# LuoweiZhou/VLP

Measured on NVIDIA H100. Metric: image_text_samples_per_sec, higher is better.
Workload: dtype bf16

## Files before the change

include/vlpk.h:

```cpp
#ifndef VLPK_H_
#define VLPK_H_

#include <stddef.h>
#include <stdint.h>

#ifdef __cplusplus
extern "C" {
#endif

#define VLPK_VERSION 102

#define VLPK_BF16 0
#define VLPK_F32 1
#define VLPK_I64 2
#define VLPK_MASK_ADDITIVE 0
#define VLPK_MASK_ZERO_ONE 1
#define VLPK_ACT_NONE 0
#define VLPK_ACT_RELU 1

typedef struct VlpkDropout {
  float p;
  uint64_t seed;
  const uint64_t* seed_dev;
} VlpkDropout;
// ... 27 lines not shown
typedef struct VlpkLayerActs {
  void* qkv;
  void* ctx;
  void* t1;
  void* y1;
  void* u;
  void* hmid;
  void* t2;
  void* y;
  float* lse;
  float* stats1;
  float* stats2;
  void* kv;
  unsigned char* drop_attn;
} VlpkLayerActs;

typedef struct VlpkBwdScratch {
  void* dz2;
  void* dt2;
  void* du;
  void* dy1;
  void* dz1;
  void* dt1;
  void* dctx;
  void* dqkv;
  void* dx;
} VlpkBwdScratch;

int vlpk_version(void);
const char* vlpk_last_error(void);
void vlpk_set_reserved_sms(int n);
void vlpk_set_deterministic(int on);
int vlpk_debug_plan_gemm(int M, int N, int K, int a_mn, int b_mn, int nseg, int seg_rows, int epi, int bn, int splits, int* out2);
int vlpk_debug_set_option(const char* name, int value);

int vlpk_mask_pack(const void* mask, int dtype, int mode, int B, int rows, int kv, int64_t stride_b, int64_t stride_r,
                   uint32_t* out, void* stream);

int vlpk_mask_synth(const int32_t* len_b, const int32_t* mode, int len_a, int B, int L, uint32_t* out, void* stream);

int vlpk_linear_fwd(int M, int N, int K, const void* x, int64_t ldx, const void* w, int64_t ldw, const void* bias, void* y,
                    int64_t ldy, int act, const VlpkDropout* drop, uint64_t site, void* stream);
int vlpk_linear_bwd(int M, int N, int K, const void* x, int64_t ldx, const void* w, int64_t ldw, const void* y, int64_t ldy,
                    const void* dy, int64_t lddy, void* dpre, void* dx, int64_t lddx, float* dw, int64_t lddw, float* db,
                    int act, float p_drop, void* stream);

int vlpk_embed_fwd(int B, int L, int H, int R, int vis_input, const int64_t* ids, const int64_t* token_type, const int64_t* pos,
                   const void* word_w, const void* pos_w, const void* type_w, const void* vis, const void* vis_pe,
                   const void* ln_g, const void* ln_b, void* y, float* stats, const VlpkDropout* drop, uint64_t site, void* stream);
int vlpk_embed_bwd(int B, int L, int H, int R, int vis_input, const int64_t* ids, const int64_t* token_type, const int64_t* pos,
                   const void* word_w, const void* pos_w, const void* type_w, const void* vis, const void* vis_pe,
                   const void* ln_g, const float* stats, const void* dy, void* dz, float* d_ln_g, float* d_ln_b,
                   const VlpkDropout* drop, uint64_t site, void* stream);

int vlpk_embed_tables_bwd(int B, int L, int H, int R, int vis_input, const int64_t* ids, const int64_t* token_type, const int64_t* pos,
                          const void* dz, int V, int P, int T, void* d_word, float* word_scratch, float* d_pos, float* d_type,
                          void* stream);

int vlpk_ln_res_drop_fwd(int64_t M, int H, const void* t, const void* res, const void* gamma, const void* beta, void* y,
                         float* stats, const VlpkDropout* drop, uint64_t site, void* stream);
int vlpk_ln_res_drop_bwd(int64_t M, int H, const void* t, const void* res, const void* gamma, const float* stats, const void* dy,
                         void* dz, void* dt, float* dgamma, float* dbeta, float* dbias, const VlpkDropout* drop, uint64_t site,
                         void* stream);

int vlpk_attn_core_fwd(int B, int heads, int Lq, int Lkv, const void* q, int64_t ld_q, const void* k, const void* v, int64_t ld_kv,
                       const uint32_t* mask_bits, int mask_rows, void* ctx, int64_t ld_ctx, float* lse, const VlpkDropout* drop,
// ... 116 lines not shown
```

vlp_b200/_lib.py:

```python
import ctypes as C
import os

import torch

_HERE = os.path.dirname(os.path.abspath(__file__))
LIB_PATH = os.path.join(_HERE, "libvlpk.so")

c_void_p, c_int, c_i64, c_u64, c_float = C.c_void_p, C.c_int, C.c_int64, C.c_uint64, C.c_float


class VlpkDropout(C.Structure):
    _fields_ = [("p", c_float), ("seed", c_u64), ("seed_dev", c_void_p)]


class VlpkShape(C.Structure):
    _fields_ = [("B", C.c_int32), ("Lq", C.c_int32), ("Lkv", C.c_int32), ("H", C.c_int32), ("heads", C.c_int32),
                ("I", C.c_int32), ("kv_slots", C.c_int32)]


WEIGHT_FIELDS = ["wq", "wk", "wv", "bq", "bk", "bv", "wo", "bo", "ln1_g", "ln1_b", "w1", "b1", "w2", "b2", "ln2_g", "ln2_b"]
GRAD_FIELDS = ["wqkv", "bqkv", "wo", "bo", "ln1_g", "ln1_b", "w1", "b1", "w2", "b2", "ln2_g", "ln2_b"]
ACT_FIELDS = ["qkv", "ctx", "t1", "y1", "u", "hmid", "t2", "y", "lse", "stats1", "stats2", "kv", "drop_attn"]
SCRATCH_FIELDS = ["dz2", "dt2", "du", "dy1", "dz1", "dt1", "dctx", "dqkv", "dx"]


class VlpkLayerWeights(C.Structure):
    _fields_ = [(n, c_void_p) for n in WEIGHT_FIELDS]


class VlpkLayerGrads(C.Structure):
    _fields_ = [(n, c_void_p) for n in GRAD_FIELDS]


class VlpkLayerActs(C.Structure):
    _fields_ = [(n, c_void_p) for n in ACT_FIELDS]


class VlpkBwdScratch(C.Structure):
    _fields_ = [(n, c_void_p) for n in SCRATCH_FIELDS]


class VlpkAdamTensor(C.Structure):
    _fields_ = [("param", c_void_p), ("grad", c_void_p), ("master", c_void_p), ("m", c_void_p), ("v", c_void_p), ("n", c_i64),
                ("weight_decay", c_float), ("param_dtype", C.c_int32), ("grad_dtype", C.c_int32), ("reserved", C.c_int32)]


_P = c_void_p
_SIGS = {
    "vlpk_version": (c_int, []),
    "vlpk_last_error": (C.c_char_p, []),
    "vlpk_debug_set_option": (c_int, [C.c_char_p, c_int]),
    "vlpk_set_reserved_sms": (None, [c_int]),
    "vlpk_set_deterministic": (None, [c_int]),
    "vlpk_debug_plan_gemm": (c_int, [c_int] * 10 + [C.POINTER(c_int)]),
    "vlpk_mask_pack": (c_int, [_P, c_int, c_int, c_int, c_int, c_int, c_i64, c_i64, _P, _P]),
    "vlpk_mask_synth": (c_int, [_P, _P, c_int, c_int, c_int, _P, _P]),
    "vlpk_linear_fwd": (c_int, [c_int, c_int, c_int, _P, c_i64, _P, c_i64, _P, _P, c_i64, c_int, C.POINTER(VlpkDropout), c_u64, _P]),
    "vlpk_linear_bwd": (c_int, [c_int, c_int, c_int, _P, c_i64, _P, c_i64, _P, c_i64, _P, c_i64, _P, _P, c_i64, _P, c_i64, _P,
                                c_int, c_float, _P]),
    "vlpk_embed_fwd": (c_int, [c_int, c_int, c_int, c_int, c_int, _P, _P, _P, _P, _P, _P, _P, _P, _P, _P, _P, _P,
                               C.POINTER(VlpkDropout), c_u64, _P]),
    "vlpk_embed_bwd": (c_int, [c_int, c_int, c_int, c_int, c_int, _P, _P, _P, _P, _P, _P, _P, _P, _P, _P, _P, _P, _P, _P,
                               C.POINTER(VlpkDropout), c_u64, _P]),
    "vlpk_embed_tables_bwd": (c_int, [c_int, c_int, c_int, c_int, c_int, _P, _P, _P, _P, c_int, c_int, c_int, _P, _P, _P, _P, _P]),
    "vlpk_ln_res_drop_fwd": (c_int, [c_i64, c_int, _P, _P, _P, _P, _P, _P, C.POINTER(VlpkDropout), c_u64, _P]),
    "vlpk_ln_res_drop_bwd": (c_int, [c_i64, c_int, _P, _P, _P, _P, _P, _P, _P, _P, _P, _P, C.POINTER(VlpkDropout), c_u64, _P]),
    "vlpk_attn_core_fwd": (c_int, [c_int, c_int, c_int, c_int, _P, c_i64, _P, _P, c_i64, _P, c_int, _P, c_i64, _P,
                                   C.POINTER(VlpkDropout), c_u64, _P]),
    "vlpk_attn_core_bwd": (c_int, [c_int, c_int, c_int, _P, _P, _P, c_i64, _P, c_int, _P, _P, c_i64, _P, _P, _P, _P, c_i64,
                                   C.POINTER(VlpkDropout), c_u64, _P]),
    "vlpk_attn_core_fwd_wide": (c_int, [c_int, c_int, c_int, c_int, _P, c_i64, _P, _P, c_i64, _P, c_int, _P, c_i64, _P,
                                        C.POINTER(VlpkDropout), c_u64, c_int, _P]),
    "vlpk_attn_core_bwd_wide": (c_int, [c_int, c_int, c_int, _P, _P, _P, c_i64, _P, c_int, _P, _P, c_i64, _P, _P, _P, _P, c_i64,
                                        C.POINTER(VlpkDropout), c_u64, c_int, _P]),
    "vlpk_attn_core_self_fwd": (c_int, [c_int, c_int, c_int, c_int, _P, c_i64, c_i64, _P, _P, c_i64, c_i64, _P, _P, _P, c_int, _P, c_i64,
                                        c_i64, _P, _P]),
    "vlpk_attn_core_group_self_fwd": (c_int, [c_int, c_int, c_int, c_int, c_int, c_int, _P, c_i64, c_i64, _P, c_int, c_i64, _P, c_int,
                                              c_i64, _P, _P, _P, c_int, _P, c_i64, c_i64, _P, _P]),
    "vlpk_attn_probs": (c_int, [c_int, c_int, c_int, c_int, c_int, _P, c_i64, c_i64, _P, c_i64, c_i64, _P, c_int, c_int, _P, _P, c_i64,
                                c_i64, _P]),
    "vlpk_mha_fwd": (c_int, [C.POINTER(VlpkShape), C.POINTER(VlpkLayerWeights), _P, _P, _P, c_int, C.POINTER(VlpkLayerActs),
                             c_float, c_float, C.POINTER(VlpkDropout), c_u64, _P]),
    "vlpk_ffn_fwd": (c_int, [C.POINTER(VlpkShape), C.POINTER(VlpkLayerWeights), C.POINTER(VlpkLayerActs), c_float,
                             C.POINTER(VlpkDropout), c_u64, _P]),
    "vlpk_layer_fwd": (c_int, [C.POINTER(VlpkShape), C.POINTER(VlpkLayerWeights), _P, _P, _P, c_int, C.POINTER(VlpkLayerActs),
                               c_float, c_float, C.POINTER(VlpkDropout), c_u64, _P]),
    "vlpk_layer_bwd": (c_int, [C.POINTER(VlpkShape), C.POINTER(VlpkLayerWeights), _P, _P, c_int, C.POINTER(VlpkLayerActs), _P, _P,
# ... 97 lines not shown
```

vlp_b200/csrc/api.cu:

```cuda
#include "../../include/vlpk.h"

#include <cstdlib>
#include <cstring>

#include "attn.cuh"
#include "decode.cuh"
#include "gemm.cuh"
#include "head.cuh"
#include "host.cuh"
#include "optim.cuh"
#include "rowops.cuh"
#include "tables.cuh"

using namespace vlpk;
typedef __nv_bfloat16 bf16;

namespace {

inline cudaStream_t S(void* s) { return reinterpret_cast<cudaStream_t>(s); }

enum { SITE_ATTN = 0, SITE_HID1 = 1, SITE_HID2 = 2 };
inline uint64_t site_of(uint64_t layer_id, int site) { return layer_id * 8 + site; }

inline DropoutCfg mk_drop(const VlpkDropout* d, float p, uint64_t site) {
// ... 372 lines not shown
  VlpkShape rows = *s;
  rows.Lq = rows.Lkv = R;
  VLPK_TRY(attn_out_ln(&rows, w, x, a, 0.f, nullptr, layer_id, st));
  return ffn_fwd_impl(&rows, w, a, 0.f, nullptr, layer_id, st);
}

int score_stack_fwd(const VlpkShape* s, int T, int n_layers, const VlpkLayerWeights* w, const void* x, AttnGroupKv* group,
                    const void* const* prefix, const uint32_t* key_bits, const uint32_t* query_bits, VlpkLayerActs* acts, cudaStream_t st) {
  const void* cur = x;
  for (int i = 0; i < n_layers; ++i) {
    if (group != nullptr) group->prefix = prefix[i];
    VLPK_TRY(score_layer_fwd(s, T, group, &w[i], cur, key_bits, query_bits, &acts[i], i, st));
    cur = acts[i].y;
  }
  return 0;
}

size_t act_bytes(const VlpkShape* s, size_t rows, size_t kv_elems) {
  const size_t H = s->H, I = s->I, M = static_cast<size_t>(s->B) * rows;
  const size_t lse = (static_cast<size_t>(s->B) * s->heads * rows + 3) / 4 * 4;
  return 2 * (M * (3 * H + 5 * H + 2 * I) + kv_elems) + 4 * (lse + 4 * M);
}

}

#pragma GCC visibility push(default)
extern "C" {

int vlpk_version(void) { return VLPK_VERSION; }
int vlpk_debug_set_option(const char* name, int value) {
  VLPK_CHECK_ARG(name != nullptr, "set_option: null name");
  if (strcmp(name, "wgrad_stream") == 0) { g_wgrad_stream = value ? 1 : 0; return 0; }
  if (strcmp(name, "attn_tiled") == 0) { set_attn_tiled(value != 0); return 0; }
  set_error("set_option: unknown option '%s'", name);
  return -1;
}
int vlpk_debug_plan_gemm(int M, int N, int K, int a_mn, int b_mn, int nseg, int seg_rows, int epi, int bn, int splits, int* out2) {
  GemmDesc g;
  g.M = M; g.N = N; g.K = K;
  g.a_mn = a_mn != 0; g.b_mn = b_mn != 0;
  g.nseg = nseg; g.b_seg_rows = seg_rows;
  g.epi = epi; g.bn = bn; g.splits = splits;
  return plan_gemm(g, &out2[0], &out2[1]);
}
void vlpk_set_reserved_sms(int n) { set_reserved_sms(n); }
void vlpk_set_deterministic(int on) { set_deterministic(on != 0); }
const char* vlpk_last_error(void) { return get_error(); }

int vlpk_mask_pack(const void* mask, int dtype, int mode, int B, int rows, int kv, int64_t stride_b, int64_t stride_r, uint32_t* out,
                   void* stream) {
  VLPK_CHECK_ARG(mask != nullptr && out != nullptr, "mask_pack: null pointer");
  return launch_mask_pack(mask, dtype, mode, B, rows, kv, stride_b, stride_r, out, S(stream));
}

int vlpk_mask_synth(const int32_t* len_b, const int32_t* mode, int len_a, int B, int L, uint32_t* out, void* stream) {
  return launch_mask_synth(len_b, mode, len_a, B, L, out, S(stream));
}

int vlpk_linear_fwd(int M, int N, int K, const void* x, int64_t ldx, const void* w, int64_t ldw, const void* bias, void* y, int64_t ldy,
                    int act, const VlpkDropout* drop, uint64_t site, void* stream) {
  VLPK_CHECK_ARG(x && w && y, "linear_fwd: null pointer");
  VLPK_CHECK_ARG(act == VLPK_ACT_NONE || act == VLPK_ACT_RELU, "linear_fwd: act %d unsupported", act);
  const DropoutCfg dc = (act == VLPK_ACT_RELU && drop != nullptr) ? mk_drop(drop, drop->p, site) : make_dropout(0.f, 0, site);
  return fwd_linear(M, N, K, x, ldx, w, ldw, bias, y, ldy, act == VLPK_ACT_RELU ? EPI_RELU : EPI_STORE, nullptr, 0, dc, S(stream));
}

int vlpk_linear_bwd(int M, int N, int K, const void* x, int64_t ldx, const void* w, int64_t ldw, const void* y, int64_t ldy,
                    const void* dy, int64_t lddy, void* dpre, void* dx, int64_t lddx, float* dw, int64_t lddw, float* db, int act,
                    float p_drop, void* stream) {
  VLPK_CHECK_ARG(x && w && dy && dw, "linear_bwd: null pointer");
  cudaStream_t st = S(stream);
  const void* g = dy;
  int64_t ldg = lddy;
  if (act == VLPK_ACT_RELU) {
    VLPK_CHECK_ARG(y != nullptr && dpre != nullptr && N % 8 == 0, "linear_bwd: relu needs y, dpre and N %% 8 == 0");
    const long long n = static_cast<long long>(M) * N;
// ... 516 lines not shown
```

vlp_b200/csrc/gemm.cu:

```cuda
#include "gemm.cuh"

#include <cstdlib>

#include "host.cuh"
#include "rowops.cuh"

namespace vlpk {

static constexpr int BM = 128;
static constexpr int BK = 64;
static constexpr int NUM_THREADS = 384;
static constexpr int PRODUCER_REGS = 24;
static constexpr int CONSUMER_REGS = 240;
static constexpr int STG_BYTES = 64 * 128;
static constexpr int STG_PER_CONSUMER = 4;
static constexpr int SMEM_MAX = 232448;
static constexpr int BN = 128;

struct GemmTmaps {
  CUtensorMap a;
  CUtensorMap b[3];
  CUtensorMap d0;
  CUtensorMap d1;
  CUtensorMap aux;
};

struct GemmArgs {
  int M, N, K;
  int b_seg_rows;
  int splits;
  int split_slices;
  const __nv_bfloat16* bias[3];
  float relu_scale;
  DropoutCfg drop;
  float* colsum;
};

template <int STAGES>
struct SmemLayout {
  static constexpr int A_BYTES = BM * BK * 2;
  static constexpr int B_BYTES = BN * BK * 2;
  static constexpr int STAGE_BYTES = A_BYTES + B_BYTES;
  static constexpr int OFF_STG = STAGES * STAGE_BYTES;
  static constexpr int OFF_BAR = OFF_STG + 2 * STG_PER_CONSUMER * STG_BYTES;
  static constexpr int NUM_BARS = 3 * STAGES + 2;
  static constexpr int TOTAL = OFF_BAR + NUM_BARS * 8;
  static constexpr int DYN_BYTES = TOTAL + 1024;
  static_assert(DYN_BYTES <= SMEM_MAX, "shared memory budget exceeded");
};

struct StageCount {
  static constexpr int value = (SMEM_MAX - 1024 - 2 * STG_PER_CONSUMER * STG_BYTES - 256) / (BM * BK * 2 + BN * BK * 2);
};

__device__ __forceinline__ void wg_bar_sync(int cw) {
  asm volatile("bar.sync %0, 128;" ::"r"(cw + 1) : "memory");
}

template <bool A_MN, bool B_MN, int EPI>
__global__ void __launch_bounds__(NUM_THREADS, 1)
gemm_kernel(const __grid_constant__ GemmTmaps tm, const GemmArgs args) {
  constexpr int STAGES = StageCount::value;
  using L = SmemLayout<STAGES>;
  extern __shared__ uint8_t smem_raw[];
  uint8_t* smem = reinterpret_cast<uint8_t*>((reinterpret_cast<uintptr_t>(smem_raw) + 1023) & ~uintptr_t(1023));

  uint64_t* bars = reinterpret_cast<uint64_t*>(smem + L::OFF_BAR);
  uint64_t* full_bar = bars;
  uint64_t* empty_bar = bars + 2 * STAGES;
  uint64_t* aux_bar = bars + 3 * STAGES;
  constexpr bool HAS_AUX = (EPI == EPI_ADD || EPI == EPI_MUL || EPI == EPI_DRELU);

  pdl_launch_dependents();
  const int wg = __shfl_sync(0xffffffffu, threadIdx.x >> 7, 0);
  const int lane = threadIdx.x & 31;

  const int num_m = (args.M + BM - 1) / BM;
  const int num_n = (args.N + BN - 1) / BN;
  const int total_kb = (args.K + BK - 1) / BK;
  const int kb_per = (total_kb + args.splits - 1) / args.splits;
  const int num_work = num_m * num_n * args.splits;

  if (threadIdx.x == 0) {
    tma_prefetch_desc(&tm.a);
    tma_prefetch_desc(&tm.b[0]);
    tma_prefetch_desc(&tm.d0);
    if (HAS_AUX) tma_prefetch_desc(&tm.aux);
    for (int i = 0; i < 2 * STAGES; ++i) mbar_init(&full_bar[i], 1);
    for (int i = 0; i < STAGES; ++i) mbar_init(&empty_bar[i], 4);
    for (int i = 0; i < 2; ++i) mbar_init(&aux_bar[i], 1);
    fence_mbar_init();
  }
  __syncthreads();
  pdl_wait();

  if (wg == 0) {
    setmaxnreg_dec<PRODUCER_REGS>();
    if (threadIdx.x < 32) {
      int stage = 0;
      uint32_t phase = 0;
      int item = 0;
      for (int w = blockIdx.x; w < num_work; w += gridDim.x, ++item) {
        uint64_t* fb = full_bar + (item & 1) * STAGES;
        const int n_blk = w % num_n;
        const int m_blk = (w / num_n) % num_m;
        const int split = w / (num_n * num_m);
        const int kb0 = split * kb_per;
        const int kb1 = min(total_kb, kb0 + kb_per);
        const int m0 = m_blk * BM;
        for (int kb = kb0; kb < kb1; ++kb) {
          mbar_wait(&empty_bar[stage], phase ^ 1u);
          if (elect_one()) {
            uint8_t* sA = smem + stage * L::STAGE_BYTES;
            uint8_t* sB = sA + L::A_BYTES;
            mbar_arrive_expect_tx(&fb[stage], L::STAGE_BYTES);
            if (!A_MN) {
              tma_load_2d(sA, &tm.a, &fb[stage], kb * BK, m0);
            } else {
#pragma unroll
              for (int j = 0; j < BM / 64; ++j) tma_load_2d(sA + j * 8192, &tm.a, &fb[stage], m0 + j * 64, kb * BK);
            }
            if (!B_MN) {
              const int n0 = n_blk * BN;
              const int seg = n0 / args.b_seg_rows;
              tma_load_2d(sB, &tm.b[seg], &fb[stage], kb * BK, n0 - seg * args.b_seg_rows);
            } else {
              const int k0 = kb * BK;
              const int seg = k0 / args.b_seg_rows;
#pragma unroll
              for (int j = 0; j < BN / 64; ++j)
                tma_load_2d(sB + j * 8192, &tm.b[seg], &fb[stage], n_blk * BN + j * 64, k0 - seg * args.b_seg_rows);
            }
          }
          __syncwarp();
          if (++stage == STAGES) {
            stage = 0;
            phase ^= 1u;
          }
        }
      }
    }
  } else {
    setmaxnreg_inc<CONSUMER_REGS>();
    const int cw = wg - 1;
    const int t = threadIdx.x - 128 * wg;
    const int fr = (t >> 5) * 16 + (lane >> 2);
    const int fc = (lane & 3) * 2;
    const bool store_thread = (t == 0);
    const uint64_t dseed = drop_seed(args.drop);
    constexpr bool HAS_BIAS = !B_MN && (EPI == EPI_STORE || EPI == EPI_GELU || EPI == EPI_RELU);
    uint8_t* stg_base = smem + L::OFF_STG + cw * STG_PER_CONSUMER * STG_BYTES;
    const uint32_t a_base = smem_u32(smem);
    const uint32_t b_base = smem_u32(smem) + L::A_BYTES;
    uint64_t* fb = full_bar + cw * STAGES;
    int stage = 0;
    uint32_t phases = 0;
    uint32_t box_seq = 0;
    uint32_t aux_phase = 0;
    bool timed_out = false;
    float acc[2][BN / 2];
#pragma unroll
    for (int i = 0; i < BN / 2; ++i) acc[0][i] = acc[1][i] = 0.f;
    for (int w = blockIdx.x + cw * gridDim.x; w < num_work; w += 2 * gridDim.x) {
      const int w_other = w - static_cast<int>(gridDim.x);
      if (w_other >= static_cast<int>(blockIdx.x)) {
        const int split_o = w_other / (num_n * num_m);
        const int kb0_o = split_o * kb_per;
        stage = (stage + min(total_kb, kb0_o + kb_per) - kb0_o) % STAGES;
      }
      const int n_blk = w % num_n;
      const int m_blk = (w / num_n) % num_m;
      const int split = w / (num_n * num_m);
      const int kb0 = split * kb_per;
      const int kb1 = min(total_kb, kb0 + kb_per);
      const int n0 = n_blk * BN;

      int prev_stage = 0;
      for (int kb = kb0; kb < kb1; ++kb) {
        mbar_wait_flag(&fb[stage], (phases >> stage) & 1u, timed_out);
        phases ^= 1u << stage;
        const uint32_t sa = a_base + stage * L::STAGE_BYTES;
        const uint32_t sb = b_base + stage * L::STAGE_BYTES;
        reg_fence(acc[0]);
        reg_fence(acc[1]);
        wgmma_fence();
#pragma unroll
        for (int k = 0; k < BK / 16; ++k) {
          const uint64_t bdesc = B_MN ? wgmma_desc_sw128(sb + k * 2048, 8192, 1024) : wgmma_desc_sw128(sb + k * 32, 16, 1024);
#pragma unroll
          for (int h = 0; h < 2; ++h) {
            const uint32_t sah = sa + h * 8192;
            const uint64_t adesc = A_MN ? wgmma_desc_sw128(sah + k * 2048, 8192, 1024) : wgmma_desc_sw128(sah + k * 32, 16, 1024);
            wgmma_m64n128k16_ss<A_MN ? 1 : 0, B_MN ? 1 : 0>(acc[h], adesc, bdesc, (kb > kb0 || k > 0) ? 1u : 0u);
          }
        }
        wgmma_commit();
        if (HAS_AUX && kb == kb0) {
          static_assert(STG_PER_CONSUMER == 2 * (BN / 64), "one staging box per aux box of a tile");
          wg_bar_sync(cw);
          if (store_thread) {
            tma_store_wait_read<0>();
            fence_proxy_async_smem();
            mbar_arrive_expect_tx(&aux_bar[cw], STG_PER_CONSUMER * STG_BYTES);
#pragma unroll
            for (int b = 0; b < STG_PER_CONSUMER; ++b)
              tma_load_2d(stg_base + b * STG_BYTES, &tm.aux, &aux_bar[cw], n0 + (b & 1) * 64, m_blk * BM + (b >> 1) * 64);
          }
        }
        wgmma_wait<1>();
        reg_fence(acc[0]);
        reg_fence(acc[1]);
        if (kb > kb0 && lane == 0) mbar_arrive(&empty_bar[prev_stage]);
        prev_stage = stage;
        if (++stage == STAGES) stage = 0;
      }
      wgmma_wait<0>();
      reg_fence(acc[0]);
      reg_fence(acc[1]);
      if (lane == 0) mbar_arrive(&empty_bar[prev_stage]);

      if (EPI == EPI_REDUCE_F32) {
        constexpr int NBOX = BN / 32;
#pragma unroll
        for (int h = 0; h < 2; ++h) {
          const int m0 = m_blk * BM + h * 64;
#pragma unroll
          for (int c = 0; c < NBOX; ++c) {
            uint8_t* stg = stg_base + (box_seq % STG_PER_CONSUMER) * STG_BYTES;
            if (store_thread) tma_store_wait_read<STG_PER_CONSUMER - 1>();
            wg_bar_sync(cw);
#pragma unroll
            for (int j = 0; j < 8; ++j) {
              const int i = c * 16 + 2 * j;
              const int r = fr + 8 * (j & 1), col = 8 * (j >> 1) + fc;
              *reinterpret_cast<float2*>(stg + r * 128 + (((col >> 2) ^ (r & 7)) << 4) + (col & 3) * 4) = make_float2(acc[h][i], acc[h][i + 1]);
            }
            fence_proxy_async_smem();
            wg_bar_sync(cw);
            if (store_thread) {
              tma_reduce_add_3d(&tm.d0, stg, n0 + c * 32, m0, args.split_slices ? split : 0);
              tma_store_commit();
            }
            ++box_seq;
          }
        }
      } else {
        constexpr int NBOX = BN / 64;
        if (HAS_AUX) {
          mbar_wait_flag(&aux_bar[cw], aux_phase, timed_out);
          aux_phase ^= 1u;
        }
        const __nv_bfloat16* bp = nullptr;
        int bias_off = 0;
        if (HAS_BIAS) {
          const int seg = n0 / args.b_seg_rows;
          bp = args.bias[seg];
          bias_off = seg * args.b_seg_rows;
        }
#pragma unroll
        for (int h = 0; h < 2; ++h) {
          const int m0 = m_blk * BM + h * 64;
          int nh = n0;
          const __nv_bfloat16* bph = bp;
          uint64_t dsh = dseed;
          asm volatile("" : "+r"(nh), "+l"(bph), "+l"(dsh));
#pragma unroll
          for (int c = 0; c < NBOX; ++c) {
            uint8_t* stg = (EPI == EPI_GELU) ? stg_base + (box_seq & 1u) * 2 * STG_BYTES : stg_base + (box_seq % STG_PER_CONSUMER) * STG_BYTES;
            uint8_t* stg_g = stg + STG_BYTES;
            if (store_thread) {
              if (EPI == EPI_GELU) tma_store_wait_read<STG_PER_CONSUMER / 2 - 1>(); else tma_store_wait_read<STG_PER_CONSUMER - 1>();
            }
            wg_bar_sync(cw);
#pragma unroll
            for (int j = 0; j < 16; ++j) {
              const int i = c * 32 + 2 * j;
              const int r = fr + 8 * (j & 1), col = 8 * (j >> 1) + fc;
              const int n = nh + c * 64 + col;
              const long long m = m0 + r;
              const int so = r * 128 + (((col >> 3) ^ (r & 7)) << 4) + (col & 7) * 2;
              float v0 = acc[h][i], v1 = acc[h][i + 1];
              if (HAS_BIAS) {
                if (bph != nullptr && n < args.N) {
                  const float2 bb = unpack_bf16x2(__ldg(reinterpret_cast<const unsigned int*>(bph + n - bias_off)));
                  v0 += bb.x;
                  v1 += bb.y;
                }
              }
              if (EPI == EPI_GELU) {
                float g0, d0, g1, d1;
                gelu_and_grad(v0, g0, d0);
                gelu_and_grad(v1, g1, d1);
                *reinterpret_cast<uint32_t*>(stg + so) = pack_bf16x2(d0, d1);
                *reinterpret_cast<uint32_t*>(stg_g + so) = pack_bf16x2(g0, g1);
                continue;
              }
              if (EPI == EPI_RELU) {
                uint32_t keep = 0xFFu;
                if (args.drop.p > 0.f)
                  keep = dropout_keep8(dsh, args.drop.site, (static_cast<uint64_t>(m) * args.N + (n - fc)) >> 3, args.drop.thresh16);
                v0 = fmaxf(v0, 0.f);
                v1 = fmaxf(v1, 0.f);
                v0 = ((keep >> fc) & 1u) ? v0 * args.drop.scale : 0.f;
                v1 = ((keep >> (fc + 1)) & 1u) ? v1 * args.drop.scale : 0.f;
// ... 10 lines not shown
                  v1 = x.y > 0.f ? v1 * args.relu_scale : 0.f;
                }
              }
              *reinterpret_cast<uint32_t*>(stg + so) = pack_bf16x2(v0, v1);
            }
            fence_proxy_async_smem();
            wg_bar_sync(cw);
            if (store_thread) {
              tma_store_2d(&tm.d0, stg, nh + c * 64, m0);
              if (EPI == EPI_GELU) tma_store_2d(&tm.d1, stg_g, nh + c * 64, m0);
              tma_store_commit();
            }
            if (EPI != EPI_GELU && args.colsum != nullptr) {
              const int col = t & 63, r0 = (t >> 6) * 32;
              float acc_c = 0.f;
#pragma unroll 8
              for (int rr = r0; rr < r0 + 32; ++rr) {
                const __nv_bfloat16 v = *reinterpret_cast<const __nv_bfloat16*>(stg + rr * 128 + (((col >> 3) ^ (rr & 7)) << 4) + (col & 7) * 2);
                acc_c += __bfloat162float(v);
              }
              if (nh + c * 64 + col < args.N) atomicAdd(args.colsum + nh + c * 64 + col, acc_c);
            }
            ++box_seq;
          }
        }
      }
    }
    if (store_thread) tma_store_wait<0>();
    if (timed_out) __trap();
  }
}

template <bool A_MN, bool B_MN, int EPI>
static int launch_inst(const GemmTmaps& tm, const GemmArgs& args, int num_work, cudaStream_t stream) {
  constexpr int STAGES = StageCount::value;
  using L = SmemLayout<STAGES>;
  auto kfn = gemm_kernel<A_MN, B_MN, EPI>;
  static bool attr_set = false;
  if (!attr_set) {
    VLPK_CUDA(cudaFuncSetAttribute(kfn, cudaFuncAttributeMaxDynamicSharedMemorySize, L::DYN_BYTES));
    attr_set = true;
  }
  const int max_ctas = gemm_sms();
  const int ctas = num_work < max_ctas ? num_work : max_ctas;
  LaunchScope scope(A_MN ? CAT_GEMM_WGRAD : (B_MN ? CAT_GEMM_DGRAD : CAT_GEMM_FWD), 2.0 * args.M * args.N * args.K, stream);
  VLPK_CUDA(launch_ex(kfn, dim3(ctas), dim3(NUM_THREADS), L::DYN_BYTES, stream, 1, tm, args));
  return 0;
}

static int dispatch(const GemmDesc& g, const GemmTmaps& tm, const GemmArgs& args, int num_work, cudaStream_t s) {
  if (!g.a_mn && !g.b_mn) {
    switch (g.epi) {
      case EPI_STORE: return launch_inst<false, false, EPI_STORE>(tm, args, num_work, s);
      case EPI_GELU: return launch_inst<false, false, EPI_GELU>(tm, args, num_work, s);
      case EPI_RELU: return launch_inst<false, false, EPI_RELU>(tm, args, num_work, s);
      default: break;
    }
  } else if (!g.a_mn && g.b_mn) {
    switch (g.epi) {
      case EPI_STORE: return launch_inst<false, true, EPI_STORE>(tm, args, num_work, s);
      case EPI_ADD: return launch_inst<false, true, EPI_ADD>(tm, args, num_work, s);
      case EPI_MUL: return launch_inst<false, true, EPI_MUL>(tm, args, num_work, s);
      case EPI_DRELU: return launch_inst<false, true, EPI_DRELU>(tm, args, num_work, s);
      case EPI_REDUCE_F32: return launch_inst<false, true, EPI_REDUCE_F32>(tm, args, num_work, s);
      default: break;
    }
  } else if (g.a_mn && g.b_mn) {
    if (g.epi == EPI_REDUCE_F32) return launch_inst<true, true, EPI_REDUCE_F32>(tm, args, num_work, s);
    if (g.epi == EPI_STORE) return launch_inst<true, true, EPI_STORE>(tm, args, num_work, s);
  }
  set_error("gemm: unsupported (a_mn=%d, b_mn=%d, epi=%d) combination", (int)g.a_mn, (int)g.b_mn, g.epi);
  return -1;
}

static double tile_cost(int M, int N, int total_kb, int splits, bool reduce) {
  const int num_m = (M + BM - 1) / BM;
  const int num_n = (N + BN - 1) / BN;
  const long long tiles = static_cast<long long>(num_m) * num_n * splits;
  const int slots = deterministic() ? num_sms() : gemm_sms();
  const long long rounds = (tiles + slots - 1) / slots;
  const int kb_per = (total_kb + splits - 1) / splits;
  const double mainloop = kb_per * (128.0 + double(BN));
  const double epi = (reduce ? 3.0 : 1.5) * BN;
  return rounds * (mainloop + epi + 60.0);
}

int plan_gemm(const GemmDesc& g, int* bn_out, int* splits_out) {
  const int seg_rows = g.nseg > 1 ? g.b_seg_rows : (g.b_mn ? g.K : g.N);
  const int total_kb = (g.K + BK - 1) / BK;
  const bool reduce = (g.epi == EPI_REDUCE_F32);
  VLPK_CHECK_ARG(g.bn == 0 || g.bn == BN, "gemm: no valid tile configuration (bn=%d; tiles are %d wide)", g.bn, BN);
  VLPK_CHECK_ARG(g.nseg == 1 || seg_rows % (g.b_mn ? BK : BN) == 0, "gemm: segment rows %d not tile aligned", seg_rows);
  int splits = 1;
  if (reduce) {
    const int max_s = total_kb / 8 > 0 ? total_kb / 8 : 1;
    if (g.splits > 0) {
      splits = g.splits < max_s ? g.splits : max_s;
    } else {
      double best = 1e300;
      for (int s = 1; s <= max_s; ++s) {
        const double c = tile_cost(g.M, g.N, total_kb, s, reduce);
        if (c < best) {
          best = c;
          splits = s;
        }
      }
    }
  }
  if (splits > total_kb) splits = total_kb;
  {
    const int kb_per = (total_kb + splits - 1) / splits;
    splits = (total_kb + kb_per - 1) / kb_per;
  }
  *bn_out = BN;
  *splits_out = splits;
  return 0;
}

int launch_gemm(const GemmDesc& g, cudaStream_t stream) {
  VLPK_CHECK_ARG(g.M > 0 && g.N > 0 && g.K > 0, "gemm: empty problem M=%d N=%d K=%d", g.M, g.N, g.K);
  VLPK_CHECK_ARG(g.N % 8 == 0, "gemm: N=%d must be a multiple of 8", g.N);
  VLPK_CHECK_ARG(g.nseg >= 1 && g.nseg <= 3, "gemm: nseg=%d", g.nseg);
  const int seg_rows = g.nseg > 1 ? g.b_seg_rows : (g.b_mn ? g.K : g.N);
  const bool reduce = (g.epi == EPI_REDUCE_F32);
  VLPK_CHECK_ARG(g.splits <= 1 || reduce, "gemm: split-K needs EPI_REDUCE_F32");
  VLPK_CHECK_ARG(g.b_rows == 0 || (g.nseg == 1 && g.b_rows <= (g.b_mn ? g.K : g.N)), "gemm: b_rows=%d needs a single B segment", g.b_rows);

  int bn = BN, splits = 1;
  VLPK_TRY(plan_gemm(g, &bn, &splits));

  GemmTmaps tm;
  memset(&tm, 0, sizeof(tm));
  if (!g.a_mn) {
    VLPK_TRY(make_tmap_2d(&tm.a, TM_BF16, g.A, g.K, g.M, g.lda, BK, BM));
  } else {
    VLPK_TRY(make_tmap_2d(&tm.a, TM_BF16, g.A, g.M, g.K, g.lda, 64, BK));
  }
  for (int s = 0; s < g.nseg; ++s) {
    if (!g.b_mn) {
      const int rows = g.nseg > 1 ? seg_rows : (g.b_rows > 0 ? g.b_rows : g.N);
      VLPK_TRY(make_tmap_2d(&tm.b[s], TM_BF16, g.B[s], g.K, rows, g.ldb, BK, bn));
    } else {
      const int rows = g.nseg > 1 ? seg_rows : (g.b_rows > 0 ? g.b_rows : g.K);
      VLPK_TRY(make_tmap_2d(&tm.b[s], TM_BF16, g.B[s], g.N, rows, g.ldb, 64, BK));
    }
  }
  for (int s = g.nseg; s < 3; ++s) tm.b[s] = tm.b[0];
  if (reduce) {
    VLPK_CHECK_ARG(g.split_stride == 0 || (g.split_stride % 4 == 0 && g.split_stride >= static_cast<int64_t>(g.M) * g.ldd0),
                   "gemm: split_stride %lld must be a multiple of 4 and cover M x ldd0", (long long)g.split_stride);
    const uint64_t dims[3] = {static_cast<uint64_t>(g.N), static_cast<uint64_t>(g.M), static_cast<uint64_t>(g.split_stride ? splits : 1)};
    const uint64_t strides[2] = {static_cast<uint64_t>(g.ldd0) * 4,
                                 static_cast<uint64_t>(g.split_stride ? g.split_stride : static_cast<int64_t>(g.M) * g.ldd0) * 4};
    const uint32_t box[3] = {32, 64, 1};
    VLPK_TRY(make_tmap(&tm.d0, TM_F32, 3, g.D0, dims, strides, box));
    tm.d1 = tm.d0;
  } else {
    VLPK_TRY(make_tmap_2d(&tm.d0, TM_BF16, g.D0, g.N, g.M, g.ldd0, 64, 64));
    if (g.epi == EPI_GELU) {
      VLPK_CHECK_ARG(g.D1 != nullptr, "gemm: EPI_GELU needs D1");
      VLPK_TRY(make_tmap_2d(&tm.d1, TM_BF16, g.D1, g.N, g.M, g.ldd1, 64, 64));
    } else {
      tm.d1 = tm.d0;
    }
  }
  VLPK_CHECK_ARG(g.colsum == nullptr || (!reduce && g.epi != EPI_GELU), "gemm: colsum fusion is for single-output bf16 epilogues");
  if (g.epi == EPI_ADD || g.epi == EPI_MUL || g.epi == EPI_DRELU) {
    VLPK_CHECK_ARG(g.aux != nullptr && (g.ld_aux % 8) == 0 && (reinterpret_cast<uintptr_t>(g.aux) & 15u) == 0,
                   "gemm: aux must be 16-byte aligned with ld %% 8 == 0");
    VLPK_TRY(make_tmap_2d(&tm.aux, TM_BF16, g.aux, g.N, g.M, g.ld_aux, 64, 64));
  } else {
    tm.aux = tm.d0;
  }

  GemmArgs a;
  a.M = g.M;
  a.N = g.N;
  a.K = g.K;
  a.b_seg_rows = seg_rows;
  a.splits = splits;
  a.split_slices = (reduce && g.split_stride > 0) ? 1 : 0;
  for (int s = 0; s < 3; ++s) a.bias[s] = (s < g.nseg) ? g.bias[s] : nullptr;
  a.relu_scale = g.relu_scale;
  a.colsum = g.colsum;
  a.drop = g.drop;

  const int num_m = (g.M + BM - 1) / BM;
  const int num_n = (g.N + bn - 1) / bn;
  const int num_work = num_m * num_n * splits;
  return dispatch(g, tm, a, num_work, stream);
}

int launch_gemm_split_slices(GemmDesc g, int slot, cudaStream_t stream) {
  VLPK_CHECK_ARG(g.epi == EPI_REDUCE_F32 && g.split_stride == 0, "gemm: split slices are for EPI_REDUCE_F32 into one D0");
  int bn = 0, splits = 1;
  VLPK_TRY(plan_gemm(g, &bn, &splits));
  if (splits == 1) return launch_gemm(g, stream);
  VLPK_CHECK_ARG(g.ldd0 == g.N, "gemm: split slices need a dense D0 (ldd0 %lld != N %d)", (long long)g.ldd0, g.N);
  const long long n = static_cast<long long>(g.M) * g.N;
  float* part = scratch_f32(slot, static_cast<size_t>(n) * splits, stream);
  if (part == nullptr) return -1;
  VLPK_CUDA(cudaMemsetAsync(part, 0, static_cast<size_t>(n) * splits * sizeof(float), stream));
  float* out = static_cast<float*>(g.D0);
  g.D0 = part;
  g.splits = splits;
  g.split_stride = n;
  VLPK_TRY(launch_gemm(g, stream));
  return launch_sum_parts(part, splits, n, out, stream);
}

}
```

vlp_b200/csrc/gemm.cuh:

```cuda
#pragma once
#include "common.cuh"

namespace vlpk {

enum Epi : int {
  EPI_STORE = 0,
  EPI_GELU = 1,
  EPI_RELU = 2,
  EPI_ADD = 3,
  EPI_MUL = 4,
  EPI_DRELU = 5,
  EPI_REDUCE_F32 = 6,
};

struct GemmDesc {
  int M = 0, N = 0, K = 0;
  bool a_mn = false;
  const void* A = nullptr;
  int64_t lda = 0;
  bool b_mn = false;
  int nseg = 1;
  const void* B[3] = {nullptr, nullptr, nullptr};
  int64_t ldb = 0;
  int b_seg_rows = 0;
  int b_rows = 0;
  const __nv_bfloat16* bias[3] = {nullptr, nullptr, nullptr};
  void* D0 = nullptr;
  int64_t ldd0 = 0;
  void* D1 = nullptr;
  int64_t ldd1 = 0;
  const __nv_bfloat16* aux = nullptr;
  int64_t ld_aux = 0;
  int epi = EPI_STORE;
  float relu_scale = 1.0f;
  DropoutCfg drop = {0.f, 1.f, 0u, 0ull, 0ull, nullptr};
  float* colsum = nullptr;
  int splits = 1;
  int64_t split_stride = 0;
  int bn = 0;
};

int launch_gemm(const GemmDesc& g, cudaStream_t stream);
int plan_gemm(const GemmDesc& g, int* bn_out, int* splits_out);
int launch_gemm_split_slices(GemmDesc g, int slot, cudaStream_t stream);

}
```

Before: 5374.

## Add cooperative 256-row tile GEMM variant for weight-gradient reduce GEMMs

Adds a cooperative kernel variant in which both consumer warpgroups share one 256-row A tile and a common B tile, instead of each warpgroup working on a separate 128-row tile. It is used for MN-major reduce-add weight-gradient GEMMs. The planner compares a cost model for the cooperative tiles against the existing one, counting whether the last round of tiles is well filled, and picks the cheaper option per shape. Sharing the B tile cuts B loads per output and improves reuse. The cost is fewer stages, less staging smem, coarser tiles that can leave SMs idle, and a hand-tuned cost model that may choose wrongly. An option switch allows forcing the old 128-row path.

```diff
diff --git a/include/vlpk.h b/include/vlpk.h
--- a/include/vlpk.h
+++ b/include/vlpk.h
@@ -83,6 +83,7 @@
 void vlpk_set_reserved_sms(int n);
 void vlpk_set_deterministic(int on);
 int vlpk_debug_plan_gemm(int M, int N, int K, int a_mn, int b_mn, int nseg, int seg_rows, int epi, int bn, int splits, int* out2);
+int vlpk_debug_plan_gemm_rows(int M, int N, int K, int a_mn, int b_mn, int epi, int splits, int* out2);
 int vlpk_debug_set_option(const char* name, int value);
 
 int vlpk_mask_pack(const void* mask, int dtype, int mode, int B, int rows, int kv, int64_t stride_b, int64_t stride_r,
diff --git a/vlp_b200/_lib.py b/vlp_b200/_lib.py
--- a/vlp_b200/_lib.py
+++ b/vlp_b200/_lib.py
@@ -53,6 +53,7 @@
     "vlpk_set_reserved_sms": (None, [c_int]),
     "vlpk_set_deterministic": (None, [c_int]),
     "vlpk_debug_plan_gemm": (c_int, [c_int] * 10 + [C.POINTER(c_int)]),
+    "vlpk_debug_plan_gemm_rows": (c_int, [c_int] * 7 + [C.POINTER(c_int)]),
     "vlpk_mask_pack": (c_int, [_P, c_int, c_int, c_int, c_int, c_int, c_i64, c_i64, _P, _P]),
     "vlpk_mask_synth": (c_int, [_P, _P, c_int, c_int, c_int, _P, _P]),
     "vlpk_linear_fwd": (c_int, [c_int, c_int, c_int, _P, c_i64, _P, c_i64, _P, _P, c_i64, c_int, C.POINTER(VlpkDropout), c_u64, _P]),
diff --git a/vlp_b200/csrc/api.cu b/vlp_b200/csrc/api.cu
--- a/vlp_b200/csrc/api.cu
+++ b/vlp_b200/csrc/api.cu
@@ -428,6 +428,7 @@
   VLPK_CHECK_ARG(name != nullptr, "set_option: null name");
   if (strcmp(name, "wgrad_stream") == 0) { g_wgrad_stream = value ? 1 : 0; return 0; }
   if (strcmp(name, "attn_tiled") == 0) { set_attn_tiled(value != 0); return 0; }
+  if (strcmp(name, "wgrad_rows128") == 0) { set_wgrad_rows128(value != 0); return 0; }
   set_error("set_option: unknown option '%s'", name);
   return -1;
 }
@@ -438,6 +439,14 @@
   g.nseg = nseg; g.b_seg_rows = seg_rows;
   g.epi = epi; g.bn = bn; g.splits = splits;
   return plan_gemm(g, &out2[0], &out2[1]);
+}
+int vlpk_debug_plan_gemm_rows(int M, int N, int K, int a_mn, int b_mn, int epi, int splits, int* out2) {
+  GemmDesc g;
+  g.M = M; g.N = N; g.K = K;
+  g.a_mn = a_mn != 0; g.b_mn = b_mn != 0;
+  g.epi = epi; g.splits = splits;
+  int bn = 0;
+  return plan_gemm(g, &bn, &out2[1], &out2[0]);
 }
 void vlpk_set_reserved_sms(int n) { set_reserved_sms(n); }
 void vlpk_set_deterministic(int on) { set_deterministic(on != 0); }
diff --git a/vlp_b200/csrc/gemm.cu b/vlp_b200/csrc/gemm.cu
--- a/vlp_b200/csrc/gemm.cu
+++ b/vlp_b200/csrc/gemm.cu
@@ -14,6 +14,7 @@
 static constexpr int CONSUMER_REGS = 240;
 static constexpr int STG_BYTES = 64 * 128;
 static constexpr int STG_PER_CONSUMER = 4;
+static constexpr int STG_COOP = 2;
 static constexpr int SMEM_MAX = 232448;
 static constexpr int BN = 128;
 
@@ -36,32 +37,31 @@
   float* colsum;
 };
 
-template <int STAGES>
+template <int TR>
 struct SmemLayout {
-  static constexpr int A_BYTES = BM * BK * 2;
+  static constexpr int STG = TR == BM ? STG_PER_CONSUMER : STG_COOP;
+  static constexpr int A_BYTES = TR * BK * 2;
   static constexpr int B_BYTES = BN * BK * 2;
   static constexpr int STAGE_BYTES = A_BYTES + B_BYTES;
+  static constexpr int STAGES = (SMEM_MAX - 1024 - 2 * STG * STG_BYTES - 256) / STAGE_BYTES;
   static constexpr int OFF_STG = STAGES * STAGE_BYTES;
-  static constexpr int OFF_BAR = OFF_STG + 2 * STG_PER_CONSUMER * STG_BYTES;
+  static constexpr int OFF_BAR = OFF_STG + 2 * STG * STG_BYTES;
   static constexpr int NUM_BARS = 3 * STAGES + 2;
   static constexpr int TOTAL = OFF_BAR + NUM_BARS * 8;
   static constexpr int DYN_BYTES = TOTAL + 1024;
   static_assert(DYN_BYTES <= SMEM_MAX, "shared memory budget exceeded");
 };
 
-struct StageCount {
-  static constexpr int value = (SMEM_MAX - 1024 - 2 * STG_PER_CONSUMER * STG_BYTES - 256) / (BM * BK * 2 + BN * BK * 2);
-};
-
 __device__ __forceinline__ void wg_bar_sync(int cw) {
   asm volatile("bar.sync %0, 128;" ::"r"(cw + 1) : "memory");
 }
 
-template <bool A_MN, bool B_MN, int EPI>
-__global__ void __launch_bounds__(NUM_THREADS, 1)
-gemm_kernel(const __grid_constant__ GemmTmaps tm, const GemmArgs args) {
-  constexpr int STAGES = StageCount::value;
-  using L = SmemLayout<STAGES>;
+template <bool A_MN, bool B_MN, int EPI, int TR>
+__device__ __forceinline__ void gemm_body(const GemmTmaps& tm, const GemmArgs args) {
+  using L = SmemLayout<TR>;
+  constexpr int STAGES = L::STAGES;
+  constexpr bool COOP = (TR == 2 * BM);
+  static_assert(TR == BM || (COOP && A_MN && EPI == EPI_REDUCE_F32), "256-row tiles are for MN-major A and reduce-add only");
   extern __shared__ uint8_t smem_raw[];
   uint8_t* smem = reinterpret_cast<uint8_t*>((reinterpret_cast<uintptr_t>(smem_raw) + 1023) & ~uintptr_t(1023));
 
@@ -75,7 +75,7 @@
   const int wg = __shfl_sync(0xffffffffu, threadIdx.x >> 7, 0);
   const int lane = threadIdx.x & 31;
 
-  const int num_m = (args.M + BM - 1) / BM;
+  const int num_m = (args.M + TR - 1) / TR;
   const int num_n = (args.N + BN - 1) / BN;
   const int total_kb = (args.K + BK - 1) / BK;
   const int kb_per = (total_kb + args.splits - 1) / args.splits;
@@ -87,7 +87,7 @@
     tma_prefetch_desc(&tm.d0);
     if (HAS_AUX) tma_prefetch_desc(&tm.aux);
     for (int i = 0; i < 2 * STAGES; ++i) mbar_init(&full_bar[i], 1);
-    for (int i = 0; i < STAGES; ++i) mbar_init(&empty_bar[i], 4);
+    for (int i = 0; i < STAGES; ++i) mbar_init(&empty_bar[i], COOP ? 8 : 4);
     for (int i = 0; i < 2; ++i) mbar_init(&aux_bar[i], 1);
     fence_mbar_init();
   }
@@ -101,13 +101,13 @@
       uint32_t phase = 0;
       int item = 0;
       for (int w = blockIdx.x; w < num_work; w += gridDim.x, ++item) {
-        uint64_t* fb = full_bar + (item & 1) * STAGES;
+        uint64_t* fb = full_bar + (COOP ? 0 : (item & 1) * STAGES);
         const int n_blk = w % num_n;
         const int m_blk = (w / num_n) % num_m;
         const int split = w / (num_n * num_m);
         const int kb0 = split * kb_per;
         const int kb1 = min(total_kb, kb0 + kb_per);
-        const int m0 = m_blk * BM;
+        const int m0 = m_blk * TR;
         for (int kb = kb0; kb < kb1; ++kb) {
           mbar_wait(&empty_bar[stage], phase ^ 1u);
           if (elect_one()) {
@@ -118,7 +118,7 @@
               tma_load_2d(sA, &tm.a, &fb[stage], kb * BK, m0);
             } else {
 #pragma unroll
-              for (int j = 0; j < BM / 64; ++j) tma_load_2d(sA + j * 8192, &tm.a, &fb[stage], m0 + j * 64, kb * BK);
+              for (int j = 0; j < TR / 64; ++j) tma_load_2d(sA + j * 8192, &tm.a, &fb[stage], m0 + j * 64, kb * BK);
             }
             if (!B_MN) {
               const int n0 = n_blk * BN;
@@ -149,10 +149,10 @@
     const bool store_thread = (t == 0);
     const uint64_t dseed = drop_seed(args.drop);
     constexpr bool HAS_BIAS = !B_MN && (EPI == EPI_STORE || EPI == EPI_GELU || EPI == EPI_RELU);
-    uint8_t* stg_base = smem + L::OFF_STG + cw * STG_PER_CONSUMER * STG_BYTES;
-    const uint32_t a_base = smem_u32(smem);
+    uint8_t* stg_base = smem + L::OFF_STG + cw * L::STG * STG_BYTES;
+    const uint32_t a_base = smem_u32(smem) + (COOP ? cw * 2 * 8192 : 0);
     const uint32_t b_base = smem_u32(smem) + L::A_BYTES;
-    uint64_t* fb = full_bar + cw * STAGES;
+    uint64_t* fb = full_bar + (COOP ? 0 : cw * STAGES);
     int stage = 0;
     uint32_t phases = 0;
     uint32_t box_seq = 0;
@@ -161,9 +161,9 @@
     float acc[2][BN / 2];
 #pragma unroll
     for (int i = 0; i < BN / 2; ++i) acc[0][i] = acc[1][i] = 0.f;
-    for (int w = blockIdx.x + cw * gridDim.x; w < num_work; w += 2 * gridDim.x) {
+    for (int w = blockIdx.x + (COOP ? 0 : cw * gridDim.x); w < num_work; w += (COOP ? 1 : 2) * gridDim.x) {
       const int w_other = w - static_cast<int>(gridDim.x);
-      if (w_other >= static_cast<int>(blockIdx.x)) {
+      if (!COOP && w_other >= static_cast<int>(blockIdx.x)) {
         const int split_o = w_other / (num_n * num_m);
         const int kb0_o = split_o * kb_per;
         stage = (stage + min(total_kb, kb0_o + kb_per) - kb0_o) % STAGES;
@@ -196,14 +196,14 @@
         }
         wgmma_commit();
         if (HAS_AUX && kb == kb0) {
-          static_assert(STG_PER_CONSUMER == 2 * (BN / 64), "one staging box per aux box of a tile");
+          static_assert(!HAS_AUX || L::STG == 2 * (BN / 64), "one staging box per aux box of a tile");
           wg_bar_sync(cw);
           if (store_thread) {
             tma_store_wait_read<0>();
             fence_proxy_async_smem();
-            mbar_arrive_expect_tx(&aux_bar[cw], STG_PER_CONSUMER * STG_BYTES);
-#pragma unroll
-            for (int b = 0; b < STG_PER_CONSUMER; ++b)
+            mbar_arrive_expect_tx(&aux_bar[cw], L::STG * STG_BYTES);
+#pragma unroll
+            for (int b = 0; b < L::STG; ++b)
               tma_load_2d(stg_base + b * STG_BYTES, &tm.aux, &aux_bar[cw], n0 + (b & 1) * 64, m_blk * BM + (b >> 1) * 64);
           }
         }
@@ -223,11 +223,11 @@
         constexpr int NBOX = BN / 32;
 #pragma unroll
         for (int h = 0; h < 2; ++h) {
-          const int m0 = m_blk * BM + h * 64;
+          const int m0 = m_blk * TR + (COOP ? cw * BM : 0) + h * 64;
 #pragma unroll
           for (int c = 0; c < NBOX; ++c) {
-            uint8_t* stg = stg_base + (box_seq % STG_PER_CONSUMER) * STG_BYTES;
-            if (store_thread) tma_store_wait_read<STG_PER_CONSUMER - 1>();
+            uint8_t* stg = stg_base + (box_seq % L::STG) * STG_BYTES;
+            if (store_thread) tma_store_wait_read<L::STG - 1>();
             wg_bar_sync(cw);
 #pragma unroll
             for (int j = 0; j < 8; ++j) {
@@ -266,10 +266,10 @@
           asm volatile("" : "+r"(nh), "+l"(bph), "+l"(dsh));
 #pragma unroll
           for (int c = 0; c < NBOX; ++c) {
-            uint8_t* stg = (EPI == EPI_GELU) ? stg_base + (box_seq & 1u) * 2 * STG_BYTES : stg_base + (box_seq % STG_PER_CONSUMER) * STG_BYTES;
+            uint8_t* stg = (EPI == EPI_GELU) ? stg_base + (box_seq & 1u) * 2 * STG_BYTES : stg_base + (box_seq % L::STG) * STG_BYTES;
             uint8_t* stg_g = stg + STG_BYTES;
             if (store_thread) {
-              if (EPI == EPI_GELU) tma_store_wait_read<STG_PER_CONSUMER / 2 - 1>(); else tma_store_wait_read<STG_PER_CONSUMER - 1>();
+              if (EPI == EPI_GELU) tma_store_wait_read<L::STG / 2 - 1>(); else tma_store_wait_read<L::STG - 1>();
             }
             wg_bar_sync(cw);
 #pragma unroll
@@ -346,10 +346,22 @@
 }
 
 template <bool A_MN, bool B_MN, int EPI>
+__global__ void __launch_bounds__(NUM_THREADS, 1)
+gemm_kernel(const __grid_constant__ GemmTmaps tm, const GemmArgs args) {
+  gemm_body<A_MN, B_MN, EPI, BM>(tm, args);
+}
+
+template <bool A_MN, bool B_MN, int EPI>
+__global__ void __launch_bounds__(NUM_THREADS, 1)
+gemm_coop_kernel(const __grid_constant__ GemmTmaps tm, const GemmArgs args) {
+  gemm_body<A_MN, B_MN, EPI, 2 * BM>(tm, args);
+}
+
+template <bool A_MN, bool B_MN, int EPI, int TR = BM>
 static int launch_inst(const GemmTmaps& tm, const GemmArgs& args, int num_work, cudaStream_t stream) {
-  constexpr int STAGES = StageCount::value;
-  using L = SmemLayout<STAGES>;
-  auto kfn = gemm_kernel<A_MN, B_MN, EPI>;
+  using L = SmemLayout<TR>;
+  void (*kfn)(const GemmTmaps, const GemmArgs);
+  if constexpr (TR == BM) kfn = gemm_kernel<A_MN, B_MN, EPI>; else kfn = gemm_coop_kernel<A_MN, B_MN, EPI>;
   static bool attr_set = false;
   if (!attr_set) {
     VLPK_CUDA(cudaFuncSetAttribute(kfn, cudaFuncAttributeMaxDynamicSharedMemorySize, L::DYN_BYTES));
@@ -362,7 +374,7 @@
   return 0;
 }
 
-static int dispatch(const GemmDesc& g, const GemmTmaps& tm, const GemmArgs& args, int num_work, cudaStream_t s) {
+static int dispatch(const GemmDesc& g, int rows, const GemmTmaps& tm, const GemmArgs& args, int num_work, cudaStream_t s) {
   if (!g.a_mn && !g.b_mn) {
     switch (g.epi) {
       case EPI_STORE: return launch_inst<false, false, EPI_STORE>(tm, args, num_work, s);
@@ -380,12 +392,16 @@
       default: break;
     }
   } else if (g.a_mn && g.b_mn) {
+    if (g.epi == EPI_REDUCE_F32 && rows == 2 * BM) return launch_inst<true, true, EPI_REDUCE_F32, 2 * BM>(tm, args, num_work, s);
     if (g.epi == EPI_REDUCE_F32) return launch_inst<true, true, EPI_REDUCE_F32>(tm, args, num_work, s);
     if (g.epi == EPI_STORE) return launch_inst<true, true, EPI_STORE>(tm, args, num_work, s);
   }
   set_error("gemm: unsupported (a_mn=%d, b_mn=%d, epi=%d) combination", (int)g.a_mn, (int)g.b_mn, g.epi);
   return -1;
 }
+
+static bool g_wgrad_rows128 = false;
+void set_wgrad_rows128(bool on) { g_wgrad_rows128 = on; }
 
 static double tile_cost(int M, int N, int total_kb, int splits, bool reduce) {
   const int num_m = (M + BM - 1) / BM;
@@ -399,17 +415,39 @@
   return rounds * (mainloop + epi + 60.0);
 }
 
-int plan_gemm(const GemmDesc& g, int* bn_out, int* splits_out) {
+static constexpr double COOP_KB = 1.54;
+static constexpr double COOP_EPI = 21.0;
+static double coop_tile_cost(int M, int N, int total_kb, int splits) {
+  const int num_m = (M + 2 * BM - 1) / (2 * BM);
+  const int num_n = (N + BN - 1) / BN;
+  const long long tiles = static_cast<long long>(num_m) * num_n * splits;
+  const int slots = deterministic() ? num_sms() : gemm_sms();
+  const long long rounds = (tiles + slots - 1) / slots;
+  const int kb_per = (total_kb + splits - 1) / splits;
+  const double mainloop = kb_per * COOP_KB * (128.0 + double(BN));
+  const double epi = COOP_EPI * BN;
+  return rounds * (mainloop + epi + 60.0);
+}
+
+static bool coop_round_filled(int M, int N, int splits) {
+  const long long tiles = static_cast<long long>((M + 2 * BM - 1) / (2 * BM)) * ((N + BN - 1) / BN) * splits;
+  const int slots = deterministic() ? num_sms() : gemm_sms();
+  return 20 * tiles >= 17 * ((tiles + slots - 1) / slots) * slots;
+}
+
+int plan_gemm(const GemmDesc& g, int* bn_out, int* splits_out, int* rows_out) {
   const int seg_rows = g.nseg > 1 ? g.b_seg_rows : (g.b_mn ? g.K : g.N);
   const int total_kb = (g.K + BK - 1) / BK;
   const bool reduce = (g.epi == EPI_REDUCE_F32);
   VLPK_CHECK_ARG(g.bn == 0 || g.bn == BN, "gemm: no valid tile configuration (bn=%d; tiles are %d wide)", g.bn, BN);
   VLPK_CHECK_ARG(g.nseg == 1 || seg_rows % (g.b_mn ? BK : BN) == 0, "gemm: segment rows %d not tile aligned", seg_rows);
-  int splits = 1;
+  const bool coop = reduce && g.a_mn && g.b_mn && !g_wgrad_rows128;
+  int splits = 1, rows = BM;
   if (reduce) {
     const int max_s = total_kb / 8 > 0 ? total_kb / 8 : 1;
     if (g.splits > 0) {
       splits = g.splits < max_s ? g.splits : max_s;
+      if (coop && coop_tile_cost(g.M, g.N, total_kb, splits) < tile_cost(g.M, g.N, total_kb, splits, reduce)) rows = 2 * BM;
     } else {
       double best = 1e300;
       for (int s = 1; s <= max_s; ++s) {
@@ -417,6 +455,13 @@
         if (c < best) {
           best = c;
           splits = s;
+          rows = BM;
+        }
+        const double cc = coop && coop_round_filled(g.M, g.N, s) ? coop_tile_cost(g.M, g.N, total_kb, s) : 1e300;
+        if (cc < best) {
+          best = cc;
+          splits = s;
+          rows = 2 * BM;
         }
       }
     }
@@ -428,6 +473,7 @@
   }
   *bn_out = BN;
   *splits_out = splits;
+  if (rows_out != nullptr) *rows_out = rows;
   return 0;
 }
 
@@ -440,8 +486,8 @@
   VLPK_CHECK_ARG(g.splits <= 1 || reduce, "gemm: split-K needs EPI_REDUCE_F32");
   VLPK_CHECK_ARG(g.b_rows == 0 || (g.nseg == 1 && g.b_rows <= (g.b_mn ? g.K : g.N)), "gemm: b_rows=%d needs a single B segment", g.b_rows);
 
-  int bn = BN, splits = 1;
-  VLPK_TRY(plan_gemm(g, &bn, &splits));
+  int bn = BN, splits = 1, rows = BM;
+  VLPK_TRY(plan_gemm(g, &bn, &splits, &rows));
 
   GemmTmaps tm;
   memset(&tm, 0, sizeof(tm));
@@ -499,10 +545,10 @@
   a.colsum = g.colsum;
   a.drop = g.drop;
 
-  const int num_m = (g.M + BM - 1) / BM;
+  const int num_m = (g.M + rows - 1) / rows;
   const int num_n = (g.N + bn - 1) / bn;
   const int num_work = num_m * num_n * splits;
-  return dispatch(g, tm, a, num_work, stream);
+  return dispatch(g, rows, tm, a, num_work, stream);
 }
 
 int launch_gemm_split_slices(GemmDesc g, int slot, cudaStream_t stream) {
diff --git a/vlp_b200/csrc/gemm.cuh b/vlp_b200/csrc/gemm.cuh
--- a/vlp_b200/csrc/gemm.cuh
+++ b/vlp_b200/csrc/gemm.cuh
@@ -41,7 +41,8 @@
 };
 
 int launch_gemm(const GemmDesc& g, cudaStream_t stream);
-int plan_gemm(const GemmDesc& g, int* bn_out, int* splits_out);
+int plan_gemm(const GemmDesc& g, int* bn_out, int* splits_out, int* rows_out = nullptr);
+void set_wgrad_rows128(bool on);
 int launch_gemm_split_slices(GemmDesc g, int slot, cudaStream_t stream);
 
 }
```

Result: faster. 5517 (median of 6 runs) (+2.7%).
